# ECP-WarpX/WarpX

Measured on AMD Instinct MI355X. Metric: particle_steps_per_s, higher is better.
Workload: dtype f64; 1 GPU; 3D uniform_plasma 256x256x256, 8 ppc, Yee FDTD, order-3 shape, esirkepov, boris, filter on; cells_per_gpu=16777216, particles_per_gpu=134217728, n_ranks=1, ranks_per_gpu=1, sort_interval=2, single_precision_comms=False, preroll_steps=40, overlap_halo=False, momentum_synchronisation=outside the timed region (the K steps are consecutive steps of one longer run)

## Files before the change

### warpx_amd/csrc/common.hpp

```cpp
#ifndef WXA_COMMON_HPP_
#define WXA_COMMON_HPP_

#include <hip/hip_runtime.h>
#include <stdint.h>
#include <stdio.h>

#include "../../include/warpx_amd.h"

#ifndef WXA_OPAQUE_F64
#define WXA_OPAQUE_F64(v) asm volatile("" : "+v"(v))
#define WXA_OPAQUE_I32(v) asm volatile("" : "+v"(v))
#endif

#ifndef WXA_WAVES_PER_SIMD
#define WXA_WAVES_PER_SIMD(n) __attribute__((amdgpu_waves_per_eu(n, n)))
#endif

namespace wxa {

namespace PhysConst {
constexpr double c = 299'792'458.;
constexpr double ep0 = 8.8541878128e-12;
constexpr double mu0 = 1.25663706212e-06;
constexpr double q_e = 1.602176634e-19;
constexpr double m_e = 9.1093837015e-31;
constexpr double r_e = 2.817940326204929e-15;
}

void set_last_error(const char* fmt, ...);

#define WXA_HIP_CHECK(expr)                                                          \
    do {                                                                             \
        hipError_t _e = (expr);                                                      \
        if (_e != hipSuccess) {                                                      \
            ::wxa::set_last_error("%s failed: %s (%s:%d)", #expr, hipGetErrorString(_e), \
                                  __FILE__, __LINE__);                               \
            return WXA_ERR_HIP;                                                      \
        }                                                                            \
    } while (0)

#define WXA_LAUNCH_CHECK()                                                           \
    do {                                                                             \
        hipError_t _e = hipGetLastError();                                           \
        if (_e != hipSuccess) {                                                      \
            ::wxa::set_last_error("kernel launch failed: %s (%s:%d)", hipGetErrorString(_e), \
                                  __FILE__, __LINE__);                               \
            return WXA_ERR_HIP;                                                      \
        }                                                                            \
    } while (0)

#define WXA_REQUIRE(cond, msg)                                                       \
    do {                                                                             \
        if (!(cond)) {                                                               \
            ::wxa::set_last_error("invalid argument: %s (%s)", msg, #cond);          \
            return WXA_ERR_INVALID_ARG;                                              \
        }                                                                            \
    } while (0)

struct DevF {
    double* __restrict__ p;
    int lo0, lo1, lo2;
    int n0, n1, n2;
    long js, ks;
    __host__ __device__ inline long off(int i, int j, int k) const {
        return (long)(i - lo0) + (long)(j - lo1) * js + (long)(k - lo2) * ks;
    }
    __device__ inline double& operator()(int i, int j, int k) const { return p[off(i, j, k)]; }
};

inline DevF make_devf(const wxa_field_view& v) {
    DevF f;
    f.p = v.p;
    f.lo0 = v.lo[0]; f.lo1 = v.lo[1]; f.lo2 = v.lo[2];
    f.n0 = v.n[0]; f.n1 = v.n[1]; f.n2 = v.n[2];
    f.js = v.jstride; f.ks = v.kstride;
    return f;
}

struct Box3 {
    int lo[3];
    int hi[3];
};

inline Box3 valid_box(const wxa_field_view& v) {
    Box3 b;
    for (int d = 0; d < 3; ++d) {
        b.lo[d] = v.lo[d] + v.ng[d];
        b.hi[d] = v.lo[d] + v.n[d] - v.ng[d];
    }
    return b;
}

inline bool is_stag(const wxa_field_view& v, int a, int b, int c) {
    return v.stag[0] == a && v.stag[1] == b && v.stag[2] == c;
}
// ... 31 lines not shown
```

### warpx_amd/csrc/gather_tile.hip

```cpp
#include "dispatch.hpp"
#include "gather_body.hpp"
#include "push_sort.hpp"
#include "tile_launch.hpp"

#include <stdlib.h>

namespace wxa {

#ifdef WXA_GATHER_PROFILE
__device__ unsigned long long wxa_gather_prof[8];
#define GPROF_CLOCK(v) const long long v = clock64()
#define GPROF_ADD(n, v) do { if (threadIdx.x == 0) atomicAdd(&wxa_gather_prof[n], (unsigned long long)(v)); } while (0)
#else
#define GPROF_CLOCK(v)
#define GPROF_ADD(n, v)
#endif

constexpr int GT_TS = WXA_TILE;
constexpr int GT_THREADS = 512;

template <int G, int O = 3>
struct GatherTileDims {
    static constexpr int LO = O == 4 ? (G ? -2 : -3) : (G ? -1 : -2);
    static constexpr int N = GT_TS + (O == 4 ? (G ? 5 : 6) : (G ? 3 : 4));
    static constexpr int NPTS = N * N * N;
};

struct SplitTile {
    static constexpr int stag(int c, int d) {
        return c == 0 ? d == 0 : c == 1 ? d == 1 : c == 2 ? d == 2 : c == 3 ? d != 0 : c == 4 ? d != 1 : d != 2;
    }
    static constexpr int n(int c, int d) { return stag(c, d) ? GT_TS + 4 : GT_TS + 3; }
    static constexpr int lo(int c, int d) { return stag(c, d) ? -2 : -1; }
    static constexpr int pts(int c) { return n(c, 0) * n(c, 1) * n(c, 2); }
    static constexpr int off(int c) { return c == 0 ? 0 : off(c - 1) + pts(c - 1); }
    static constexpr int total() { return off(6); }
};

template <int N>
struct LdsField {
    const double* base;
    __device__ __forceinline__ const double* at(int i, int j, int k) const { return base + i + N * (j + N * k); }
    static constexpr long js = N, ks = N * N;
};

template <int PUSHER, bool MOVE>
__device__ __forceinline__ void push_and_store(const PV& p, int ip, double xp, double yp, double zp, double ux, double uy,
                                               double uz, double Exp, double Eyp, double Ezp, double Bxp, double Byp,
                                               double Bzp, double q, double m, double dt, const ExtEB& ext,
                                               const PushSort& hook,
                                               int* lds_hist = nullptr, const long my_tile = -1) {
    add_external_fields(ext, ip, Exp, Eyp, Ezp, Bxp, Byp, Bzp);
    push_momentum<PUSHER>(ux, uy, uz, Exp, Eyp, Ezp, Bxp, Byp, Bzp, q, m, dt);
    if constexpr (MOVE) update_position(xp, yp, zp, ux, uy, uz, dt);
    if constexpr (MOVE) {
        if (!push_sort_tail(hook, p, ip, xp, yp, zp, ux, uy, uz, lds_hist, my_tile)) return;
    }
    p.ux[ip] = ux; p.uy[ip] = uy; p.uz[ip] = uz;
    if constexpr (MOVE) { p.x[ip] = xp; p.y[ip] = yp; p.z[ip] = zp; }
}

template <int O, int G, int PUSHER, bool MOVE, int PART = 0>
__global__ void __launch_bounds__(GT_THREADS) WXA_WAVES_PER_SIMD(O <= 3 ? 4 : 2)
gather_push_tile_kernel(PV p, const int* __restrict__ offsets, DevF Ex, DevF Ey, DevF Ez, DevF Bx, DevF By,
                        DevF Bz, Geom g, TileGeom tg, double q, double m, double dt, StragglerQueue sq, ExtEB ext,
                        PushSort hook, HeavyUnits hu) {
    constexpr int N = GatherTileDims<G, O>::N;
    constexpr int NPTS = GatherTileDims<G, O>::NPTS;
    constexpr bool SPLIT = G == 0 && O <= 3;
    __shared__ double F[SPLIT ? SplitTile::total() : 6 * NPTS];
    const long ntiles = (long)tg.nt[0] * tg.nt[1] * tg.nt[2];
    if (blockIdx.x == 0 && threadIdx.x == 0 && sq.next) *sq.next = 0u;
    long tile;
    int unit_u, unit_k;
    if (!heavy_unit_of(hu, blockIdx.x, ntiles, tile, unit_u, unit_k)) return;
    constexpr int TC = GT_TS * GT_TS * GT_TS;
    int start = offsets[tile * TC];
    int end = offsets[(tile + 1) * TC];
    if (unit_k > 1) {
        const long chunks = ((long)(end - start) + 63) >> 6;
        const int s0 = start;
        start = s0 + (int)((chunks * unit_u / unit_k) << 6);
        end = min(end, s0 + (int)((chunks * (unit_u + 1) / unit_k) << 6));
    }
    if (end <= start) return;
    const int tid = threadIdx.x;
    GPROF_CLOCK(prof_t0);
    const int ti = (int)(tile % tg.nt[0]);
    const int tj = (int)((tile / tg.nt[0]) % tg.nt[1]);
    const int tk = (int)(tile / ((long)tg.nt[0] * tg.nt[1]));
    if constexpr (PART != 0) {
        const bool face = ti == 0 || ti == tg.nt[0] - 1 || tj == 0 || tj == tg.nt[1] - 1 || tk == 0 || tk == tg.nt[2] - 1;
        if (face != (PART == 2)) return;
    }
    const int o0 = tg.cell_lo[0] + ti * GT_TS + GatherTileDims<G, O>::LO;
    const int o1 = tg.cell_lo[1] + tj * GT_TS + GatherTileDims<G, O>::LO;
    const int o2 = tg.cell_lo[2] + tk * GT_TS + GatherTileDims<G, O>::LO;
    static_assert(GT_THREADS == PUSH_SORT_TILE_CELLS, "one lane per cell of the tile");
    __shared__ int lhist[MOVE ? PUSH_SORT_TILE_CELLS : 1];
    const bool count_local = MOVE && (hook.mode & PUSH_SORT_COUNT) != 0 && unit_u == 0;
    if constexpr (MOVE) {
        if (count_local) lhist[tid] = 0;
    }
    constexpr int SCAP = 512;
    __shared__ int slist[SCAP];
    __shared__ int sn, sbase;
    if (tid == 0) sn = 0;
    auto push_straggler = [&](const int i) {
        const int n = atomicAdd(&sn, 1);
        if (n < SCAP) slist[n] = i;
        else sq.push(i);
    };
    constexpr int WAVES = GT_THREADS / 64;
    __shared__ int next_chunk;
    const int lane = tid & 63;
    int cb_next = start + 64 * __builtin_amdgcn_readfirstlane(tid >> 6) + GT_THREADS;
    if (tid == 0) next_chunk = 2 * WAVES;
    int ip = start + tid;
    double nxt[3] = {0.0, 0.0, 0.0};
    auto load_particle = [&](const int i) {
        asm volatile("" ::: "memory");
        nxt[0] = p.x[i]; nxt[1] = p.y[i]; nxt[2] = p.z[i];
        asm volatile("" ::: "memory");
    };
    if (ip < end) load_particle(ip);
    constexpr int PER = (NPTS + GT_THREADS - 1) / GT_THREADS;
    auto fetch = [&](const DevF& f, double (&r)[PER]) {
#pragma unroll
        for (int n = 0; n < PER; ++n) {
            const int a = tid + n * GT_THREADS;
            const int i = o0 + a % N, j = o1 + (a / N) % N, k = o2 + a / (N * N);
            const bool in = a < NPTS && i >= f.lo0 && i < f.lo0 + f.n0 && j >= f.lo1 && j < f.lo1 + f.n1 && k >= f.lo2 &&
                            k < f.lo2 + f.n2;
            r[n] = in ? f.p[f.off(i, j, k)] : 0.0;
        }
    };
    auto put = [&](int c, const double (&r)[PER]) {
#pragma unroll
        for (int n = 0; n < PER; ++n) {
            const int a = tid + n * GT_THREADS;
            if (a < NPTS) F[c * NPTS + a] = r[n];
        }
    };
    if constexpr (SPLIT) {
        const int t0 = o0 - GatherTileDims<G, O>::LO, t1 = o1 - GatherTileDims<G, O>::LO, t2 = o2 - GatherTileDims<G, O>::LO;
        constexpr int PERS = (SplitTile::pts(3) + GT_THREADS - 1) / GT_THREADS;
        auto fetch_c = [&](auto cc, const DevF& f, double (&r)[PERS]) {
            constexpr int c = decltype(cc)::value, n0 = SplitTile::n(c, 0), n1 = SplitTile::n(c, 1);
#pragma unroll
            for (int n = 0; n < PERS; ++n) {
                const int a = tid + n * GT_THREADS;
                const int i = t0 + SplitTile::lo(c, 0) + a % n0, j = t1 + SplitTile::lo(c, 1) + (a / n0) % n1,
                          k = t2 + SplitTile::lo(c, 2) + a / (n0 * n1);
                const bool in = a < SplitTile::pts(c) && i >= f.lo0 && i < f.lo0 + f.n0 && j >= f.lo1 && j < f.lo1 + f.n1 &&
                                k >= f.lo2 && k < f.lo2 + f.n2;
                r[n] = in ? f.p[f.off(i, j, k)] : 0.0;
            }
        };
        auto put_c = [&](auto cc, const double (&r)[PERS]) {
            constexpr int c = decltype(cc)::value;
#pragma unroll
            for (int n = 0; n < PERS; ++n) {
                const int a = tid + n * GT_THREADS;
                if (a < SplitTile::pts(c)) F[SplitTile::off(c) + a] = r[n];
            }
        };
        using std::integral_constant;
        double r0[PERS], r1[PERS], r2[PERS], r3[PERS], r4[PERS], r5[PERS];
        fetch_c(integral_constant<int, 0>{}, Ex, r0); fetch_c(integral_constant<int, 1>{}, Ey, r1); fetch_c(integral_constant<int, 2>{}, Ez, r2);
        fetch_c(integral_constant<int, 3>{}, Bx, r3); fetch_c(integral_constant<int, 4>{}, By, r4); fetch_c(integral_constant<int, 5>{}, Bz, r5);
        put_c(integral_constant<int, 0>{}, r0); put_c(integral_constant<int, 1>{}, r1); put_c(integral_constant<int, 2>{}, r2);
        put_c(integral_constant<int, 3>{}, r3); put_c(integral_constant<int, 4>{}, r4); put_c(integral_constant<int, 5>{}, r5);
    } else {
        double r0[PER], r1[PER], r2[PER], r3[PER], r4[PER], r5[PER];
        fetch(Ex, r0); fetch(Ey, r1); fetch(Ez, r2); fetch(Bx, r3); fetch(By, r4); fetch(Bz, r5);
        put(0, r0); put(1, r1); put(2, r2); put(3, r3); put(4, r4); put(5, r5);
    }
    __syncthreads();
    GPROF_CLOCK(prof_t1);
    GPROF_ADD(0, prof_t1 - prof_t0);
    GPROF_ADD(2, 1);

    int claimed = 0;
    auto advance = [&]() {
        ip = cb_next + lane;
        cb_next = start + 64 * __builtin_amdgcn_readfirstlane(__shfl(claimed, 0));
    };
    for (; ip < end; advance()) {
        GPROF_CLOCK(prof_a);
        double xp = nxt[0], yp = nxt[1], zp = nxt[2], ux0, uy0, uz0;
        asm volatile("" ::: "memory");
        ux0 = p.ux[ip]; uy0 = p.uy[ip]; uz0 = p.uz[ip];
        asm volatile("" ::: "memory");
        if (lane == 0) claimed = atomicAdd(&next_chunk, 1);
        if (cb_next + lane < end) load_particle(cb_next + lane);
#ifdef WXA_GATHER_PROFILE
        asm volatile("s_waitcnt vmcnt(0)" : "+v"(xp), "+v"(yp), "+v"(zp));
#endif
        GPROF_CLOCK(prof_b);
        GatherShapes<O, G> s;
        gather_shapes<O, G>(xp, yp, zp, g, s);
        constexpr int NN = O + 1, NC = O + 1 - G;
        const int lo_i = min(s.jn, s.jc) - o0, hi_i = max(s.jn + NN, s.jc + NC) - 1 - o0;
        const int lo_j = min(s.kn, s.kc) - o1, hi_j = max(s.kn + NN, s.kc + NC) - 1 - o1;
        const int lo_k = min(s.ln, s.lc) - o2, hi_k = max(s.ln + NN, s.lc + NC) - 1 - o2;
        bool staged = lo_i >= 0 && lo_j >= 0 && lo_k >= 0 && hi_i < N && hi_j < N && hi_k < N;
        if constexpr (SPLIT) {
            staged = staged && s.jn - o0 >= 1 && s.kn - o1 >= 1 && s.ln - o2 >= 1;
        }
        if (!staged) {
            push_straggler(ip);
            continue;
        }
        const int jn = s.jn - o0, jc = s.jc - o0, kn = s.kn - o1, kc = s.kc - o1, ln = s.ln - o2, lc = s.lc - o2;
        double Exp, Eyp, Ezp, Bxp, Byp, Bzp;
        if constexpr (SPLIT) {
            auto rows = [&](auto cc, auto nx, auto ny, auto nz, const int i, const int j, const int k, const double* sx_,
                            const double* sy_, const double* sz_) {
                constexpr int c = decltype(cc)::value, n0 = SplitTile::n(c, 0), n1 = SplitTile::n(c, 1);
                const double* b_ = F + SplitTile::off(c) + (i - (SplitTile::lo(c, 0) + 2)) +
                                   n0 * ((j - (SplitTile::lo(c, 1) + 2)) + n1 * (k - (SplitTile::lo(c, 2) + 2)));
                return gather_rows_lds<decltype(nx)::value, decltype(ny)::value, decltype(nz)::value, n0, n0 * n1, 2>(b_, sx_, sy_, sz_);
            };
            using std::integral_constant;
            constexpr integral_constant<int, NN> nn{};
            constexpr integral_constant<int, NC> nc{};
            Exp = rows(integral_constant<int, 0>{}, nc, nn, nn, jc, kn, ln, s.sxc, s.syn, s.szn);
            Eyp = rows(integral_constant<int, 1>{}, nn, nc, nn, jn, kc, ln, s.sxn, s.syc, s.szn);
            Ezp = rows(integral_constant<int, 2>{}, nn, nn, nc, jn, kn, lc, s.sxn, s.syn, s.szc);
            Bzp = rows(integral_constant<int, 5>{}, nc, nc, nn, jc, kc, ln, s.sxc, s.syc, s.szn);
            Byp = rows(integral_constant<int, 4>{}, nc, nn, nc, jc, kn, lc, s.sxc, s.syn, s.szc);
            Bxp = rows(integral_constant<int, 3>{}, nn, nc, nc, jn, kc, lc, s.sxn, s.syc, s.szc);
        } else {
#define GROWS(...)                                                                                         \
    [&](const double* b_, const double* sx_, const double* sy_, const double* sz_) {                       \
         \
                                                                            \
        if constexpr (O <= 3) return gather_rows_lds<__VA_ARGS__, N, N * N, 2>(b_, sx_, sy_, sz_);        \
        else return gather_rows<__VA_ARGS__>(b_, N, N * N, sx_, sy_, sz_);                                 \
    }
            Exp = GROWS(NC, NN, NN)(F + 0 * NPTS + jc + N * (kn + N * ln), s.sxc, s.syn, s.szn);
            Eyp = GROWS(NN, NC, NN)(F + 1 * NPTS + jn + N * (kc + N * ln), s.sxn, s.syc, s.szn);
            Ezp = GROWS(NN, NN, NC)(F + 2 * NPTS + jn + N * (kn + N * lc), s.sxn, s.syn, s.szc);
            Bzp = GROWS(NC, NC, NN)(F + 5 * NPTS + jc + N * (kc + N * ln), s.sxc, s.syc, s.szn);
            Byp = GROWS(NC, NN, NC)(F + 4 * NPTS + jc + N * (kn + N * lc), s.sxc, s.syn, s.szc);
            Bxp = GROWS(NN, NC, NC)(F + 3 * NPTS + jn + N * (kc + N * lc), s.sxn, s.syc, s.szc);
#undef GROWS
        }
#ifdef WXA_GATHER_PROFILE
        double prof_e = Exp + Bxp;
        asm volatile("s_waitcnt lgkmcnt(0)" : "+v"(prof_e));
#endif
        GPROF_CLOCK(prof_c);
        push_and_store<PUSHER, MOVE>(p, ip, xp, yp, zp, ux0, uy0, uz0, Exp, Eyp, Ezp, Bxp, Byp, Bzp, q, m, dt, ext, hook,
                                     count_local ? lhist : nullptr, tile);
#ifdef WXA_GATHER_PROFILE
        asm volatile("s_waitcnt vmcnt(0)" ::: "memory");
        GPROF_CLOCK(prof_d);
        GPROF_ADD(3, prof_b - prof_a); GPROF_ADD(4, prof_c - prof_b); GPROF_ADD(5, prof_d - prof_c); GPROF_ADD(6, 1);
        if (prof_e == 1.2345e-300) p.x[ip] = prof_e;
#endif
    }
#ifdef WXA_GATHER_PROFILE
    { GPROF_CLOCK(prof_t2); GPROF_ADD(1, prof_t2 - prof_t1); }
#endif
    {
        __syncthreads();
        const int n = min(sn, SCAP);
        if (tid == 0 && n > 0) sbase = (int)atomicAdd(sq.count, (unsigned)n);
        __syncthreads();
        for (int i = tid; i < n; i += GT_THREADS) sq.idx[sbase + i] = slist[i];
    }
    if constexpr (MOVE) {
        if (count_local) {
            __syncthreads();
            push_sort_tile_finish(hook, lhist, tile, tid);
        }
    }
}

template <int O, int G, int PUSHER, bool MOVE>
__global__ void __launch_bounds__(256)
gather_push_stragglers_kernel(PV p, const int* __restrict__ idx, const unsigned* __restrict__ count, DevF Ex,
                              DevF Ey, DevF Ez, DevF Bx, DevF By, DevF Bz, Geom g, double q, double m, double dt,
                              ExtEB ext, PushSort hook) {
    const unsigned n = *count;
    for (unsigned t = blockIdx.x * blockDim.x + threadIdx.x; t < n; t += gridDim.x * blockDim.x) {
        const int ip = idx[t];
        const double xp = p.x[ip], yp = p.y[ip], zp = p.z[ip];
        GatherShapes<O, G> s;
        gather_shapes<O, G>(xp, yp, zp, g, s);
        double Exp, Eyp, Ezp, Bxp, Byp, Bzp;
        gather_global<O, G>(s, Ex, Ey, Ez, Bx, By, Bz, Exp, Eyp, Ezp, Bxp, Byp, Bzp);
        push_and_store<PUSHER, MOVE>(p, ip, xp, yp, zp, p.ux[ip], p.uy[ip], p.uz[ip], Exp, Eyp, Ezp, Bxp, Byp, Bzp, q, m, dt,
                                     ext, hook);
    }
}

wxa_status gather_push_tiled(const wxa_particle_view* p, const wxa_field_view E[3], const wxa_field_view B[3],
                             const wxa_grid_geom* geom, double q, double m, double dt, int order, int galerkin,
                             int pusher, bool move, int part, wxa_workspace* ws, hipStream_t st) {
    TileLaunch tl;
    wxa_status rc;
    if ((rc = plan_tile_launch(ws, (long)p->np, 16, ws->gather_flips, st, tl)) != WXA_OK) return rc;
    const PV pv = make_pv(*p);
    const Geom g = make_geom(*geom);
    const DevF ex = make_devf(E[0]), ey = make_devf(E[1]), ez = make_devf(E[2]);
    const DevF bx = make_devf(B[0]), by = make_devf(B[1]), bz = make_devf(B[2]);
    const ExtEB ext = ext_of(ws);
    const PushSort hook = make_push_sort(ws, 0, move);
    with_int<0, 1, 2, 3>(move ? 1 + part : 0, [&](auto what) {
    with_int<WXA_PUSHER_BORIS, WXA_PUSHER_VAY, WXA_PUSHER_HC, WXA_PUSHER_BORIS_RR>(pusher, [&](auto pu) {
    with_int<1, 2, 3, 4>(order, [&](auto o) {
    with_int<1, 0>(galerkin, [&](auto gk) {
        constexpr int O = decltype(o)::value, G = decltype(gk)::value, PUSHER = decltype(pu)::value;
        constexpr bool MOVE = decltype(what)::value != 0;
        constexpr int PART = MOVE ? decltype(what)::value - 1 : 0;
        hipLaunchKernelGGL((gather_push_tile_kernel<O, G, PUSHER, MOVE, PART>), dim3(tl.groups), dim3(GT_THREADS), 0, st, pv,
                           tl.offsets, ex, ey, ez, bx, by, bz, g, tl.tg, q, m, dt, tl.sq, ext, hook, tl.hu);
        hipLaunchKernelGGL((gather_push_stragglers_kernel<O, G, PUSHER, MOVE>), dim3(WXA_STRAGGLER_BLOCKS), dim3(256), 0, st,
                           pv, tl.sq.idx, tl.sq.count, ex, ey, ez, bx, by, bz, g, q, m, dt, ext, hook);
    }); }); }); });
    WXA_LAUNCH_CHECK();
    return WXA_OK;
}

}

#ifdef WXA_GATHER_PROFILE
extern "C" int wxa_debug_gather_profile(unsigned long long* out, int reset) {
    if (out && hipMemcpyFromSymbol(out, HIP_SYMBOL(wxa::wxa_gather_prof), sizeof(wxa::wxa_gather_prof)) != hipSuccess)
        return -1;
    if (reset) {
        unsigned long long z[8] = {};
        if (hipMemcpyToSymbol(HIP_SYMBOL(wxa::wxa_gather_prof), z, sizeof(z)) != hipSuccess) return -1;
    }
    return 0;
}
#endif
```

### warpx_amd/csrc/particles.hip

```cpp
#include "deposit_body.hpp"
#include <complex>

#include "dispatch.hpp"
#include "gather_body.hpp"
#include "push_sort.hpp"
#include "workspace.hpp"

#include <hipcub/hipcub.hpp>

namespace wxa {

template <int O, int G, int PUSHER, bool MOVE>
__global__ void __launch_bounds__(256)
gather_push_kernel(PV p, DevF Ex, DevF Ey, DevF Ez, DevF Bx, DevF By, DevF Bz, Geom g, double q,
                   double m, double dt, ExtEB ext, PushSort hook) {
    const long ip = (long)blockIdx.x * blockDim.x + threadIdx.x;
    if (ip >= p.np) return;
    double xp = p.x[ip], yp = p.y[ip], zp = p.z[ip];
    GatherShapes<O, G> s;
    gather_shapes<O, G>(xp, yp, zp, g, s);
    double Exp, Eyp, Ezp, Bxp, Byp, Bzp;
    gather_global<O, G>(s, Ex, Ey, Ez, Bx, By, Bz, Exp, Eyp, Ezp, Bxp, Byp, Bzp);

    add_external_fields(ext, ip, Exp, Eyp, Ezp, Bxp, Byp, Bzp);
    double ux = p.ux[ip], uy = p.uy[ip], uz = p.uz[ip];
    push_momentum<PUSHER>(ux, uy, uz, Exp, Eyp, Ezp, Bxp, Byp, Bzp, q, m, dt);
    if constexpr (MOVE) {
        update_position(xp, yp, zp, ux, uy, uz, dt);
        if (!push_sort_tail(hook, p, ip, xp, yp, zp, ux, uy, uz)) return;
        p.x[ip] = xp; p.y[ip] = yp; p.z[ip] = zp;
    }
    p.ux[ip] = ux; p.uy[ip] = uy; p.uz[ip] = uz;
}

__global__ void __launch_bounds__(256) lens_fields_kernel(PV p, ExtLens L, double* __restrict__ out, long stride) {
    const long ip = (long)blockIdx.x * blockDim.x + threadIdx.x;
    if (ip >= p.np) return;
    double Ex = 0., Ey = 0., Bx = 0., By = 0.;
    add_lens_fields(L, p.x[ip], p.y[ip], p.z[ip], p.ux[ip], p.uy[ip], p.uz[ip], Ex, Ey, Bx, By);
    out[ip] = Ex; out[stride + ip] = Ey; out[2 * stride + ip] = Bx; out[3 * stride + ip] = By;
}

template <int O>
__global__ void __launch_bounds__(256)
deposit_esirkepov_global_kernel(PV p, DevF Jx, DevF Jy, DevF Jz, Geom g, double q, EsirkepovStep es) {
    const long ip = (long)blockIdx.x * blockDim.x + threadIdx.x;
    if (ip >= p.np) return;
    const ParticleState ps{p.x[ip], p.y[ip], p.z[ip], p.w[ip], p.ux[ip], p.uy[ip], p.uz[ip]};
    EsirkepovShapes<O> s;
    esirkepov_shapes<O>(ps, g, q, es, s);
    GlobalSink sink = make_global_sink(Jx, Jy, Jz);
    sink.bi = s.bi; sink.bj = s.bj; sink.bk = s.bk;
    esirkepov_accumulate<O>(s, es, sink);
}

template <int O>
__global__ void __launch_bounds__(256)
deposit_direct_global_kernel(PV p, DevF Jx, DevF Jy, DevF Jz, Geom g, double q, double relative_time) {
    const long ip = (long)blockIdx.x * blockDim.x + threadIdx.x;
    if (ip >= p.np) return;
    const ParticleState ps{p.x[ip], p.y[ip], p.z[ip], p.w[ip], p.ux[ip], p.uy[ip], p.uz[ip]};
    DirectShapes<O> s;
    direct_shapes<O>(ps, g, q, relative_time, s);
    GlobalSink sink = make_global_sink(Jx, Jy, Jz);
    direct_accumulate<O>(s, sink);
}

template <int O>
__global__ void __launch_bounds__(256)
deposit_charge_kernel(PV p, DevF rho, int s0, int s1, int s2, Geom g, double q) {
    const long ip = (long)blockIdx.x * blockDim.x + threadIdx.x;
    if (ip >= p.np) return;
    const double invvol = g.dxi * g.dyi * g.dzi;
    const double wq = q * p.w[ip] * invvol;
    const double x = (p.x[ip] - g.xmin) * g.dxi;
    const double y = (p.y[ip] - g.ymin) * g.dyi;
    const double z = (p.z[ip] - g.zmin) * g.dzi;
    double sx[O + 1], sy[O + 1], sz[O + 1];
    const int i = g.lo0 + shape_factor<O>(sx, s0 ? x : x - 0.5);
    const int j = g.lo1 + shape_factor<O>(sy, s1 ? y : y - 0.5);
    const int k = g.lo2 + shape_factor<O>(sz, s2 ? z : z - 0.5);
    double* __restrict__ r = rho.p + rho.off(i, j, k);
#pragma unroll
    for (int iz = 0; iz <= O; iz++)
#pragma unroll
        for (int iy = 0; iy <= O; iy++)
#pragma unroll
            for (int ix = 0; ix <= O; ix++)
                atomic_add_f64(r + ix + iy * rho.js + iz * rho.ks, sx[ix] * sy[iy] * sz[iz] * wq);
}

__device__ __forceinline__ double wrap_periodic(double v, double plo, double phi) {
    const double L = phi - plo;
    if (v >= phi) {
        v -= L;
        if (v < plo) v = plo;
    } else if (v < plo) {
        v += L;
        if (v >= phi) v = nextafter(phi, plo);
    }
    return v;
}

struct PeriodicBox {
    double plo[3], phi[3];
    int on[3];
};

__global__ void __launch_bounds__(256)
enforce_periodic_kernel(double* __restrict__ x, double* __restrict__ y, double* __restrict__ z, long np,
                        PeriodicBox pb) {
    const long ip = (long)blockIdx.x * blockDim.x + threadIdx.x;
// ... 1023 lines not shown
```

### warpx_amd/csrc/push_sort.hpp

```cpp
#ifndef WXA_PUSH_SORT_HPP_
#define WXA_PUSH_SORT_HPP_

#include "gather_body.hpp"
#include "workspace.hpp"

namespace wxa {

struct SortGeom {
    double plo[3];
    double dinv[3];
    int nc[3];
    int retired_bin;
    int wrap[3] = {0, 0, 0};
};

__device__ __forceinline__ int cell_of(const SortGeom& s, double x, double y, double z) {
    int i = (int)floor((x - s.plo[0]) * s.dinv[0]);
    int j = (int)floor((y - s.plo[1]) * s.dinv[1]);
    int k = (int)floor((z - s.plo[2]) * s.dinv[2]);
    if (s.wrap[0]) i = i < 0 ? i + s.nc[0] : (i >= s.nc[0] ? i - s.nc[0] : i);
    if (s.wrap[1]) j = j < 0 ? j + s.nc[1] : (j >= s.nc[1] ? j - s.nc[1] : j);
    if (s.wrap[2]) k = k < 0 ? k + s.nc[2] : (k >= s.nc[2] ? k - s.nc[2] : k);
    i = min(max(i, 0), s.nc[0] - 1);
    j = min(max(j, 0), s.nc[1] - 1);
    k = min(max(k, 0), s.nc[2] - 1);
    constexpr int T = WXA_TILE;
    const int nti = (s.nc[0] + T - 1) / T, ntj = (s.nc[1] + T - 1) / T;
    const int tile = (i / T) + nti * ((j / T) + ntj * (k / T));
    const int kt = k % T;
    return tile * (T * T * T) + (i % T) + T * ((kt & 1) + 2 * ((j % T) + T * (kt >> 1)));
}

constexpr int PUSH_SORT_COUNT = WXA_PUSH_SORT_COUNT, PUSH_SORT_SCATTER = WXA_PUSH_SORT_SCATTER;
constexpr int PUSH_SORT_TILE_CELLS = WXA_TILE * WXA_TILE * WXA_TILE;
constexpr unsigned long long PUSH_SORT_FOREIGN = 0x80000000ull;

struct PushSort {
    int mode = 0;
    int check_retired = 0;
    double predict_dt = 0.0;
    long first = 0;
    SortGeom sg{};
    unsigned long long* __restrict__ kr_out = nullptr;
    int* __restrict__ hist = nullptr;
    int* __restrict__ fcnt = nullptr;
    int* __restrict__ own_out = nullptr;
    const unsigned long long* __restrict__ kr_in = nullptr;
    const int* __restrict__ offs = nullptr;
    const int* __restrict__ own_in = nullptr;
    double* __restrict__ dx = nullptr; double* __restrict__ dy = nullptr; double* __restrict__ dz = nullptr;
    double* __restrict__ dw = nullptr;
    double* __restrict__ dux = nullptr; double* __restrict__ duy = nullptr; double* __restrict__ duz = nullptr;
    unsigned long long* __restrict__ did = nullptr;
    long np_counted = 0;
    long n_appended = 0;
    int retired_bin_in = 0;
};

__device__ __forceinline__ long push_sort_dest(const PushSort& h, const long gi, bool& dropped) {
    dropped = false;
    if (gi >= h.np_counted) return (long)h.offs[h.retired_bin_in] + (gi - h.np_counted);
    const unsigned long long kr = h.kr_in[gi];
    const int key = (int)(kr >> 32);
    long d = (long)h.offs[key] + (long)(unsigned)(kr & 0x7fffffffull);
    if (kr & PUSH_SORT_FOREIGN) d += h.own_in[key];
    if (key == h.retired_bin_in) { d += h.n_appended; dropped = true; }
    return d;
}

__device__ __forceinline__ bool push_sort_tail(const PushSort& h, const PV& p, const long ip, const double xp, const double yp,
                                               const double zp, const double ux, const double uy, const double uz,
                                               int* lds_hist = nullptr, const long my_tile = -1) {
    if (h.mode == 0) return true;
    const long gi = h.first + ip;
    long at = gi;
    bool in_place = true;
    const bool scatter = (h.mode & PUSH_SORT_SCATTER) != 0;
    unsigned long long pid = 0ull;
    if (p.id && (scatter || h.check_retired)) pid = p.id[ip];
    bool dropped = false;
    if (scatter) {
        const double w = p.w[ip];
        at = push_sort_dest(h, gi, dropped);
        h.dx[at] = xp; h.dy[at] = yp; h.dz[at] = zp; h.dw[at] = w;
        h.dux[at] = ux; h.duy[at] = uy; h.duz[at] = uz;
        if (p.id && h.did) h.did[at] = pid;
        in_place = false;
    }
    if ((h.mode & PUSH_SORT_COUNT) && !dropped) {
        double kx = xp, ky = yp, kz = zp;
        if (h.predict_dt != 0.0) {
            constexpr double inv_c2 = 1.0 / (PhysConst::c * PhysConst::c);
            const double s_ = h.predict_dt / sqrt(1.0 + (ux * ux + uy * uy + uz * uz) * inv_c2);
            kx += ux * s_; ky += uy * s_; kz += uz * s_;
        }
        const int key = (h.check_retired && p.id && pid == WXA_IDCPU_RETIRED) ? h.sg.retired_bin : cell_of(h.sg, kx, ky, kz);
        unsigned long long rank;
        if (lds_hist && key / PUSH_SORT_TILE_CELLS == my_tile) {
            rank = (unsigned long long)(unsigned)atomicAdd(&lds_hist[key % PUSH_SORT_TILE_CELLS], 1);
        } else {
            rank = PUSH_SORT_FOREIGN | (unsigned long long)(unsigned)atomicAdd(&h.fcnt[key], 1);
            atomicAdd(&h.hist[key], 1);
        }
        h.kr_out[at] = ((unsigned long long)(unsigned)key << 32) | rank;
    }
    return in_place;
}

__device__ __forceinline__ void push_sort_tile_finish(const PushSort& h, const int* lds_hist, const long my_tile, const int tid) {
    const int n = lds_hist[tid];
    if (n > 0) {
        atomicAdd(&h.hist[my_tile * PUSH_SORT_TILE_CELLS + tid], n);
        h.own_out[my_tile * PUSH_SORT_TILE_CELLS + tid] = n;
    }
}

inline PushSort make_push_sort(const wxa_workspace* ws, const long first, const bool move) {
    PushSort h{};
    if (!ws || !move || ws->ps.armed == 0) return h;
    const auto& s = ws->ps;
    h.mode = s.armed;
    h.first = first;
    if (s.armed & PUSH_SORT_COUNT) {
        for (int d = 0; d < 3; ++d) { h.sg.plo[d] = s.plo[d]; h.sg.dinv[d] = s.dinv[d]; h.sg.nc[d] = s.nc[d]; h.sg.wrap[d] = s.wrap[d]; }
        h.sg.retired_bin = (int)s.bins;
        h.check_retired = s.check_retired;
        h.predict_dt = s.predict_dt;
        h.kr_out = (unsigned long long*)s.kr[s.out].p;
        h.hist = (int*)s.hist.p;
        h.fcnt = (int*)s.hist.p + (s.bins + 2);
        h.own_out = (int*)s.own[s.out].p;
    }
    if (s.armed & PUSH_SORT_SCATTER) {
        h.kr_in = (const unsigned long long*)s.kr[s.in].p;
        h.offs = (const int*)s.offs[s.in].p;
        h.own_in = (const int*)s.own[s.in].p;
        h.dx = s.dst.x; h.dy = s.dst.y; h.dz = s.dst.z; h.dw = s.dst.w;
        h.dux = s.dst.ux; h.duy = s.dst.uy; h.duz = s.dst.uz;
        h.did = (unsigned long long*)s.dst.idcpu;
        h.np_counted = s.pending_np;
        h.n_appended = s.appended;
        h.retired_bin_in = (int)s.pending_bins;
    }
    return h;
}

}
#endif
```

### warpx_amd/csrc/shapes.hpp

```cpp
#ifndef WXA_SHAPES_HPP_
#define WXA_SHAPES_HPP_

#include "common.hpp"

namespace wxa {

#define WXA_BSPLINE_BODY                                                   \
    if constexpr (ORDER == 0) {                                            \
        s[0] = 1.0;                                                        \
    } else if constexpr (ORDER == 1) {                                     \
        s[0] = 1.0 - xi;                                                   \
        s[1] = xi;                                                         \
    } else if constexpr (ORDER == 2) {                                     \
        s[0] = 0.5 * (0.5 - xi) * (0.5 - xi);                              \
        s[1] = 0.75 - xi * xi;                                             \
        s[2] = 0.5 * (0.5 + xi) * (0.5 + xi);                              \
    } else if constexpr (ORDER == 3) {                                     \
        const double om = 1.0 - xi;                                        \
        s[0] = (1.0 / 6.0) * om * om * om;                                 \
        s[1] = (2.0 / 3.0) - xi * xi * (1.0 - xi / 2.0);                   \
        s[2] = (2.0 / 3.0) - om * om * (1.0 - 0.5 * om);                   \
        s[3] = (1.0 / 6.0) * xi * xi * xi;                                 \
    } else {                     \
        static_assert(ORDER == 4, "orders 0..4");                          \
// ... 111 lines not shown
}

__device__ __forceinline__ void push_hc(double& ux, double& uy, double& uz, const double Ex, const double Ey,
                                        const double Ez, const double Bx, const double By, const double Bz,
                                        const double q, const double m, const double dt) {
    const double qmt = 0.5 * q * dt / m;
    constexpr double invclight = 1. / PhysConst::c;
    constexpr double invclightsq = 1. / (PhysConst::c * PhysConst::c);
    const double umx = ux + qmt * Ex, umy = uy + qmt * Ey, umz = uz + qmt * Ez;
    double gamma = 1. + (umx * umx + umy * umy + umz * umz) * invclightsq;
    const double betax = qmt * Bx, betay = qmt * By, betaz = qmt * Bz;
    const double betam = betax * betax + betay * betay + betaz * betaz;
    const double sigma = gamma - betam;
    const double ust = (umx * betax + umy * betay + umz * betaz) * invclight;
    gamma = 1. / sqrt(0.5 * (sigma + sqrt(sigma * sigma + 4. * (betam + ust * ust))));
    const double tx = gamma * betax, ty = gamma * betay, tz = gamma * betaz;
    const double s = 1. / (1. + (tx * tx + ty * ty + tz * tz));
    const double umt = umx * tx + umy * ty + umz * tz;
    const double upx = s * (umx + umt * tx + umy * tz - umz * ty);
    const double upy = s * (umy + umt * ty + umz * tx - umx * tz);
    const double upz = s * (umz + umt * tz + umx * ty - umy * tx);
    ux = upx + qmt * Ex + upy * tz - upz * ty;
    uy = upy + qmt * Ey + upz * tx - upx * tz;
    uz = upz + qmt * Ez + upx * ty - upy * tx;
}

__device__ __forceinline__ void push_boris_rr(double& ux, double& uy, double& uz, const double Ex, const double Ey,
                                              const double Ez, const double Bx, const double By, const double Bz,
                                              const double q, const double m, const double dt) {
    const double ux_old = ux, uy_old = uy, uz_old = uz;
    constexpr double inv_c2 = 1. / (PhysConst::c * PhysConst::c);
    push_boris(ux, uy, uz, Ex, Ey, Ez, Bx, By, Bz, q, m, dt);
    const double ux_n = (ux + ux_old) * 0.5;
    const double uy_n = (uy + uy_old) * 0.5;
    const double uz_n = (uz + uz_old) * 0.5;
    const double gamma_n = sqrt(1. + (ux_n * ux_n + uy_n * uy_n + uz_n * uz_n) * inv_c2);
    const double inv_gamma_n = 1.0 / gamma_n;
    const double vx_n = ux_n * inv_gamma_n;
    const double vy_n = uy_n * inv_gamma_n;
    const double vz_n = uz_n * inv_gamma_n;
    const double bx_n = vx_n / PhysConst::c;
    const double by_n = vy_n / PhysConst::c;
    const double bz_n = vz_n / PhysConst::c;
    const double flx_q = (Ex + vy_n * Bz - vz_n * By);
    const double fly_q = (Ey + vz_n * Bx - vx_n * Bz);
    const double flz_q = (Ez + vx_n * By - vy_n * Bx);
    const double fl_q2 = flx_q * flx_q + fly_q * fly_q + flz_q * flz_q;
    const double bdotE = (bx_n * Ex + by_n * Ey + bz_n * Ez);
    const double bdotE2 = bdotE * bdotE;
    const double coeff = gamma_n * gamma_n * (fl_q2 - bdotE2);
    const double q_over_mc = q / (m * PhysConst::c);
    const double RRcoeff = (2.0 / 3.0) * PhysConst::r_e * q_over_mc * q_over_mc;
    const double frx = RRcoeff * (PhysConst::c * (fly_q * Bz - flz_q * By) + bdotE * Ex - coeff * bx_n);
    const double fry = RRcoeff * (PhysConst::c * (flz_q * Bx - flx_q * Bz) + bdotE * Ey - coeff * by_n);
    const double frz = RRcoeff * (PhysConst::c * (flx_q * By - fly_q * Bx) + bdotE * Ez - coeff * bz_n);
    ux += frx * dt;
    uy += fry * dt;
    uz += frz * dt;
}

template <int PUSHER>
__device__ __forceinline__ void push_momentum(double& ux, double& uy, double& uz, const double Ex, const double Ey,
                                              const double Ez, const double Bx, const double By, const double Bz,
                                              const double q, const double m, const double dt) {
    if constexpr (PUSHER == WXA_PUSHER_BORIS) push_boris(ux, uy, uz, Ex, Ey, Ez, Bx, By, Bz, q, m, dt);
    else if constexpr (PUSHER == WXA_PUSHER_VAY) push_vay(ux, uy, uz, Ex, Ey, Ez, Bx, By, Bz, q, m, dt);
    else if constexpr (PUSHER == WXA_PUSHER_HC) push_hc(ux, uy, uz, Ex, Ey, Ez, Bx, By, Bz, q, m, dt);
    else push_boris_rr(ux, uy, uz, Ex, Ey, Ez, Bx, By, Bz, q, m, dt);
}

struct ExtLens {
    int n;
    double period, time, dt, gamma_boost, uz_boost;
    const double* tab;
};
struct ExtPerParticle {
    const double* fields;
    long stride;
};
struct ExtEB {
    double ex, ey, ez, bx, by, bz;
    ExtPerParticle pp;
};
__device__ __forceinline__ void add_external_fields(const ExtEB& ext, long ip, double& Ex, double& Ey, double& Ez, double& Bx,
                                                    double& By, double& Bz) {
    Ex += ext.ex; Ey += ext.ey; Ez += ext.ez; Bx += ext.bx; By += ext.by; Bz += ext.bz;
    WXA_OPAQUE_F64(Ex); WXA_OPAQUE_F64(Ey); WXA_OPAQUE_F64(Ez); WXA_OPAQUE_F64(Bx); WXA_OPAQUE_F64(By); WXA_OPAQUE_F64(Bz);
    if (ext.pp.fields) {
        Ex += ext.pp.fields[ip];
        Ey += ext.pp.fields[ext.pp.stride + ip];
        Bx += ext.pp.fields[2 * ext.pp.stride + ip];
        By += ext.pp.fields[3 * ext.pp.stride + ip];
    }
}

__device__ __forceinline__ void add_lens_fields(const ExtLens& L, const double x, const double y, const double z,
                                                const double ux, const double uy, const double uz, double& fEx,
                                                double& fEy, double& fBx, double& fBy) {
    constexpr double inv_c2 = 1. / (PhysConst::c * PhysConst::c);
    const double gamma = sqrt(1. + (ux * ux + uy * uy + uz * uz) * inv_c2);
    const double vzp = uz / gamma;
    double zl = z, zr = z + vzp * L.dt;
    if (L.gamma_boost > 1.) {
        zl = L.gamma_boost * zl + L.uz_boost * L.time;
        zr = L.gamma_boost * zr + L.uz_boost * (L.time + L.dt);
    }
    double Ex = 0., Ey = 0., Bx = 0., By = 0.;
    if (zl > 0) {
        const int i_lens = (int)floor(zl / L.period);
        if (i_lens < L.n) {
            const double lens_start = L.tab[i_lens] + i_lens * L.period;
            const double lens_end = lens_start + L.tab[L.n + i_lens];
            const double zl_bounded = fmin(fmax(zl, lens_start), lens_end);
            const double zr_bounded = fmin(fmax(zr, lens_start), lens_end);
            const double frac = (zr - zl) == 0. ? 1. : (zr_bounded - zl_bounded) / (zr - zl);
            const double sE = L.tab[2 * L.n + i_lens], sB = L.tab[3 * L.n + i_lens];
            Ex = x * frac * sE;
            Ey = y * frac * sE;
            Bx = +y * frac * sB;
            By = -x * frac * sB;
        }
    }
    if (L.gamma_boost > 1.) {
        const double Ex_boost = L.gamma_boost * Ex - L.uz_boost * By;
        const double Ey_boost = L.gamma_boost * Ey + L.uz_boost * Bx;
        const double Bx_boost = L.gamma_boost * Bx + L.uz_boost * Ey * inv_c2;
        const double By_boost = L.gamma_boost * By - L.uz_boost * Ex * inv_c2;
        Ex = Ex_boost; Ey = Ey_boost; Bx = Bx_boost; By = By_boost;
    }
    fEx += Ex; fEy += Ey; fBx += Bx; fBy += By;
}

__device__ __forceinline__ void update_position(double& x, double& y, double& z, const double ux,
                                                const double uy, const double uz, const double dt) {
    constexpr double inv_c2 = 1. / (PhysConst::c * PhysConst::c);
    const double inv_gamma = inv_sqrt(1. + (ux * ux + uy * uy + uz * uz) * inv_c2);
    x += ux * inv_gamma * dt;
    y += uy * inv_gamma * dt;
    z += uz * inv_gamma * dt;
}

struct Geom {
    double xmin, ymin, zmin;
    double dxi, dyi, dzi;
    int lo0, lo1, lo2;
};
inline Geom make_geom(const wxa_grid_geom& g) {
    return Geom{g.xyzmin[0], g.xyzmin[1], g.xyzmin[2], g.dinv[0], g.dinv[1], g.dinv[2], g.lo[0], g.lo[1], g.lo[2]};
}

}
#endif
```

Baseline: 10.51 billion particle-steps/s.

## Load rarely-used tile kernel args late from kernarg segment and specialize sort mode

Moves the external-field, straggler-queue and push-sort hook arguments of the gather/push tile kernel into a struct read through the kernarg segment pointer, loaded where used and hidden behind an opaque scalar-register barrier. The aim is to stop the compiler from hoisting these uniform values into scalar registers for the whole kernel, which reduces register pressure. It also adds a compile-time MODE parameter so the plain-push variant drops the sort tail entirely. In exchange it adds repeated scalar loads inside the particle loop, a tag check that traps on mismatch, and another template dimension that doubles the number of kernel instantiations.

```diff
diff --git a/warpx_amd/csrc/common.hpp b/warpx_amd/csrc/common.hpp
--- a/warpx_amd/csrc/common.hpp
+++ b/warpx_amd/csrc/common.hpp
@@ -11,6 +11,16 @@
 #define WXA_OPAQUE_F64(v) asm volatile("" : "+v"(v))
 #define WXA_OPAQUE_I32(v) asm volatile("" : "+v"(v))
 #endif
+
+#ifndef WXA_LATE_KERNARG
+#define WXA_LATE_KERNARG(T, first_param) ((const __attribute__((address_space(4))) T*)__builtin_amdgcn_kernarg_segment_ptr())
+#define WXA_OPAQUE_UNIFORM_PTR(p) asm volatile("" : "+s"(p))
+#else
+#define WXA_OPAQUE_UNIFORM_PTR(p) ((void)0)
+#endif
+
+constexpr unsigned long long WXA_LATE_TAG = 0x57584131004c4154ull;
+#define WXA_LATE_CHECK(p) do { if ((p)->late_tag != WXA_LATE_TAG) __builtin_trap(); } while (0)
 
 #ifndef WXA_WAVES_PER_SIMD
 #define WXA_WAVES_PER_SIMD(n) __attribute__((amdgpu_waves_per_eu(n, n)))
diff --git a/warpx_amd/csrc/gather_tile.hip b/warpx_amd/csrc/gather_tile.hip
--- a/warpx_amd/csrc/gather_tile.hip
+++ b/warpx_amd/csrc/gather_tile.hip
@@ -44,33 +44,52 @@
     static constexpr long js = N, ks = N * N;
 };
 
-template <int PUSHER, bool MOVE>
+template <int PUSHER, bool MOVE, int MODE, class E, class H>
 __device__ __forceinline__ void push_and_store(const PV& p, int ip, double xp, double yp, double zp, double ux, double uy,
                                                double uz, double Exp, double Eyp, double Ezp, double Bxp, double Byp,
-                                               double Bzp, double q, double m, double dt, const ExtEB& ext,
-                                               const PushSort& hook,
+                                               double Bzp, double q, double m, double dt, const E* ext,
+                                               const H* hook,
                                                int* lds_hist = nullptr, const long my_tile = -1) {
     add_external_fields(ext, ip, Exp, Eyp, Ezp, Bxp, Byp, Bzp);
     push_momentum<PUSHER>(ux, uy, uz, Exp, Eyp, Ezp, Bxp, Byp, Bzp, q, m, dt);
     if constexpr (MOVE) update_position(xp, yp, zp, ux, uy, uz, dt);
-    if constexpr (MOVE) {
-        if (!push_sort_tail(hook, p, ip, xp, yp, zp, ux, uy, uz, lds_hist, my_tile)) return;
+    if constexpr (MOVE && MODE != 0) {
+        if (!push_sort_tail<MODE>(hook, p, ip, xp, yp, zp, ux, uy, uz, lds_hist, my_tile)) return;
     }
     p.ux[ip] = ux; p.uy[ip] = uy; p.uz[ip] = uz;
     if constexpr (MOVE) { p.x[ip] = xp; p.y[ip] = yp; p.z[ip] = zp; }
 }
 
-template <int O, int G, int PUSHER, bool MOVE, int PART = 0>
+template <bool SORT>
+struct TileLateArgs {
+    unsigned long long late_tag = WXA_LATE_TAG;
+    ExtEB ext;
+    StragglerQueue sq;
+    PushSort hook;
+};
+template <>
+struct TileLateArgs<false> {
+    unsigned long long late_tag = WXA_LATE_TAG;
+    ExtEB ext;
+    StragglerQueue sq;
+};
+template <int O, int G, int PUSHER, bool MOVE, int PART = 0, int MODE = 0>
 __global__ void __launch_bounds__(GT_THREADS) WXA_WAVES_PER_SIMD(O <= 3 ? 4 : 2)
-gather_push_tile_kernel(PV p, const int* __restrict__ offsets, DevF Ex, DevF Ey, DevF Ez, DevF Bx, DevF By,
-                        DevF Bz, Geom g, TileGeom tg, double q, double m, double dt, StragglerQueue sq, ExtEB ext,
-                        PushSort hook, HeavyUnits hu) {
+gather_push_tile_kernel(TileLateArgs<MODE != 0> late_args, PV p, const int* __restrict__ offsets, DevF Ex, DevF Ey, DevF Ez,
+                        DevF Bx, DevF By, DevF Bz, Geom g, TileGeom tg, double q, double m, double dt, HeavyUnits hu) {
+    static_assert(MOVE || MODE == 0, "the sort is folded into pushes that move the particles");
+    static_assert(MODE == 0 || MODE == PUSH_SORT_RUNTIME, "a plain push, or the mode the hook names");
+    const auto late = WXA_LATE_KERNARG(TileLateArgs<MODE != 0>, late_args);
+    WXA_LATE_CHECK(late);
     constexpr int N = GatherTileDims<G, O>::N;
     constexpr int NPTS = GatherTileDims<G, O>::NPTS;
     constexpr bool SPLIT = G == 0 && O <= 3;
     __shared__ double F[SPLIT ? SplitTile::total() : 6 * NPTS];
     const long ntiles = (long)tg.nt[0] * tg.nt[1] * tg.nt[2];
-    if (blockIdx.x == 0 && threadIdx.x == 0 && sq.next) *sq.next = 0u;
+    if (blockIdx.x == 0 && threadIdx.x == 0) {
+        unsigned* const next = late->sq.next;
+        if (next) *next = 0u;
+    }
     long tile;
     int unit_u, unit_k;
     if (!heavy_unit_of(hu, blockIdx.x, ntiles, tile, unit_u, unit_k)) return;
@@ -98,7 +117,8 @@
     const int o2 = tg.cell_lo[2] + tk * GT_TS + GatherTileDims<G, O>::LO;
     static_assert(GT_THREADS == PUSH_SORT_TILE_CELLS, "one lane per cell of the tile");
     __shared__ int lhist[MOVE ? PUSH_SORT_TILE_CELLS : 1];
-    const bool count_local = MOVE && (hook.mode & PUSH_SORT_COUNT) != 0 && unit_u == 0;
+    bool count_local = false;
+    if constexpr (MODE != 0) count_local = (late->hook.mode & PUSH_SORT_COUNT) != 0 && unit_u == 0;
     if constexpr (MOVE) {
         if (count_local) lhist[tid] = 0;
     }
@@ -106,10 +126,10 @@
     __shared__ int slist[SCAP];
     __shared__ int sn, sbase;
     if (tid == 0) sn = 0;
-    auto push_straggler = [&](const int i) {
+    auto push_straggler = [&](const int i, const auto* la) {
         const int n = atomicAdd(&sn, 1);
         if (n < SCAP) slist[n] = i;
-        else sq.push(i);
+        else la->sq.idx[atomicAdd(la->sq.count, 1u)] = i;
     };
     constexpr int WAVES = GT_THREADS / 64;
     __shared__ int next_chunk;
@@ -187,6 +207,8 @@
         cb_next = start + 64 * __builtin_amdgcn_readfirstlane(__shfl(claimed, 0));
     };
     for (; ip < end; advance()) {
+        auto la = late;
+        WXA_OPAQUE_UNIFORM_PTR(la);
         GPROF_CLOCK(prof_a);
         double xp = nxt[0], yp = nxt[1], zp = nxt[2], ux0, uy0, uz0;
         asm volatile("" ::: "memory");
@@ -209,7 +231,7 @@
             staged = staged && s.jn - o0 >= 1 && s.kn - o1 >= 1 && s.ln - o2 >= 1;
         }
         if (!staged) {
-            push_straggler(ip);
+            push_straggler(ip, la);
             continue;
         }
         const int jn = s.jn - o0, jc = s.jc - o0, kn = s.kn - o1, kc = s.kc - o1, ln = s.ln - o2, lc = s.lc - o2;
@@ -252,8 +274,12 @@
         asm volatile("s_waitcnt lgkmcnt(0)" : "+v"(prof_e));
 #endif
         GPROF_CLOCK(prof_c);
-        push_and_store<PUSHER, MOVE>(p, ip, xp, yp, zp, ux0, uy0, uz0, Exp, Eyp, Ezp, Bxp, Byp, Bzp, q, m, dt, ext, hook,
-                                     count_local ? lhist : nullptr, tile);
+        if constexpr (MODE != 0)
+            push_and_store<PUSHER, MOVE, MODE>(p, ip, xp, yp, zp, ux0, uy0, uz0, Exp, Eyp, Ezp, Bxp, Byp, Bzp, q, m, dt, &la->ext,
+                                               &la->hook, count_local ? lhist : nullptr, tile);
+        else
+            push_and_store<PUSHER, MOVE, 0>(p, ip, xp, yp, zp, ux0, uy0, uz0, Exp, Eyp, Ezp, Bxp, Byp, Bzp, q, m, dt, &la->ext,
+                                            (const PushSort*)nullptr);
 #ifdef WXA_GATHER_PROFILE
         asm volatile("s_waitcnt vmcnt(0)" ::: "memory");
         GPROF_CLOCK(prof_d);
@@ -267,14 +293,15 @@
     {
         __syncthreads();
         const int n = min(sn, SCAP);
-        if (tid == 0 && n > 0) sbase = (int)atomicAdd(sq.count, (unsigned)n);
+        if (tid == 0 && n > 0) sbase = (int)atomicAdd(late->sq.count, (unsigned)n);
         __syncthreads();
-        for (int i = tid; i < n; i += GT_THREADS) sq.idx[sbase + i] = slist[i];
+        int* const sq_idx = late->sq.idx;
+        for (int i = tid; i < n; i += GT_THREADS) sq_idx[sbase + i] = slist[i];
     }
     if constexpr (MOVE) {
         if (count_local) {
             __syncthreads();
-            push_sort_tile_finish(hook, lhist, tile, tid);
+            if constexpr (MODE != 0) push_sort_tile_finish(&late->hook, lhist, tile, tid);
         }
     }
 }
@@ -292,8 +319,8 @@
         gather_shapes<O, G>(xp, yp, zp, g, s);
         double Exp, Eyp, Ezp, Bxp, Byp, Bzp;
         gather_global<O, G>(s, Ex, Ey, Ez, Bx, By, Bz, Exp, Eyp, Ezp, Bxp, Byp, Bzp);
-        push_and_store<PUSHER, MOVE>(p, ip, xp, yp, zp, p.ux[ip], p.uy[ip], p.uz[ip], Exp, Eyp, Ezp, Bxp, Byp, Bzp, q, m, dt,
-                                     ext, hook);
+        push_and_store<PUSHER, MOVE, PUSH_SORT_RUNTIME>(p, ip, xp, yp, zp, p.ux[ip], p.uy[ip], p.uz[ip], Exp, Eyp, Ezp, Bxp,
+                                                        Byp, Bzp, q, m, dt, &ext, &hook);
     }
 }
 
@@ -309,6 +336,7 @@
     const DevF bx = make_devf(B[0]), by = make_devf(B[1]), bz = make_devf(B[2]);
     const ExtEB ext = ext_of(ws);
     const PushSort hook = make_push_sort(ws, 0, move);
+    with_int<0, PUSH_SORT_RUNTIME>(hook.mode != 0 ? PUSH_SORT_RUNTIME : 0, [&](auto md) {
     with_int<0, 1, 2, 3>(move ? 1 + part : 0, [&](auto what) {
     with_int<WXA_PUSHER_BORIS, WXA_PUSHER_VAY, WXA_PUSHER_HC, WXA_PUSHER_BORIS_RR>(pusher, [&](auto pu) {
     with_int<1, 2, 3, 4>(order, [&](auto o) {
@@ -316,11 +344,16 @@
         constexpr int O = decltype(o)::value, G = decltype(gk)::value, PUSHER = decltype(pu)::value;
         constexpr bool MOVE = decltype(what)::value != 0;
         constexpr int PART = MOVE ? decltype(what)::value - 1 : 0;
-        hipLaunchKernelGGL((gather_push_tile_kernel<O, G, PUSHER, MOVE, PART>), dim3(tl.groups), dim3(GT_THREADS), 0, st, pv,
-                           tl.offsets, ex, ey, ez, bx, by, bz, g, tl.tg, q, m, dt, tl.sq, ext, hook, tl.hu);
+        constexpr int MODE = MOVE ? decltype(md)::value : 0;
+        TileLateArgs<MODE != 0> late;
+        late.ext = ext;
+        late.sq = tl.sq;
+        if constexpr (MODE != 0) late.hook = hook;
+        hipLaunchKernelGGL((gather_push_tile_kernel<O, G, PUSHER, MOVE, PART, MODE>), dim3(tl.groups), dim3(GT_THREADS), 0, st,
+                           late, pv, tl.offsets, ex, ey, ez, bx, by, bz, g, tl.tg, q, m, dt, tl.hu);
         hipLaunchKernelGGL((gather_push_stragglers_kernel<O, G, PUSHER, MOVE>), dim3(WXA_STRAGGLER_BLOCKS), dim3(256), 0, st,
                            pv, tl.sq.idx, tl.sq.count, ex, ey, ez, bx, by, bz, g, q, m, dt, ext, hook);
-    }); }); }); });
+    }); }); }); }); });
     WXA_LAUNCH_CHECK();
     return WXA_OK;
 }
diff --git a/warpx_amd/csrc/particles.hip b/warpx_amd/csrc/particles.hip
--- a/warpx_amd/csrc/particles.hip
+++ b/warpx_amd/csrc/particles.hip
@@ -27,7 +27,7 @@
     push_momentum<PUSHER>(ux, uy, uz, Exp, Eyp, Ezp, Bxp, Byp, Bzp, q, m, dt);
     if constexpr (MOVE) {
         update_position(xp, yp, zp, ux, uy, uz, dt);
-        if (!push_sort_tail(hook, p, ip, xp, yp, zp, ux, uy, uz)) return;
+        if (!push_sort_tail<PUSH_SORT_RUNTIME>(&hook, p, ip, xp, yp, zp, ux, uy, uz)) return;
         p.x[ip] = xp; p.y[ip] = yp; p.z[ip] = zp;
     }
     p.ux[ip] = ux; p.uy[ip] = uy; p.uz[ip] = uz;
diff --git a/warpx_amd/csrc/push_sort.hpp b/warpx_amd/csrc/push_sort.hpp
--- a/warpx_amd/csrc/push_sort.hpp
+++ b/warpx_amd/csrc/push_sort.hpp
@@ -14,22 +14,25 @@
     int wrap[3] = {0, 0, 0};
 };
 
-__device__ __forceinline__ int cell_of(const SortGeom& s, double x, double y, double z) {
-    int i = (int)floor((x - s.plo[0]) * s.dinv[0]);
-    int j = (int)floor((y - s.plo[1]) * s.dinv[1]);
-    int k = (int)floor((z - s.plo[2]) * s.dinv[2]);
-    if (s.wrap[0]) i = i < 0 ? i + s.nc[0] : (i >= s.nc[0] ? i - s.nc[0] : i);
-    if (s.wrap[1]) j = j < 0 ? j + s.nc[1] : (j >= s.nc[1] ? j - s.nc[1] : j);
-    if (s.wrap[2]) k = k < 0 ? k + s.nc[2] : (k >= s.nc[2] ? k - s.nc[2] : k);
-    i = min(max(i, 0), s.nc[0] - 1);
-    j = min(max(j, 0), s.nc[1] - 1);
-    k = min(max(k, 0), s.nc[2] - 1);
+template <class SG>
+__device__ __forceinline__ int cell_of_at(const SG* s, double x, double y, double z) {
+    const int nc0 = s->nc[0], nc1 = s->nc[1], nc2 = s->nc[2];
+    int i = (int)floor((x - s->plo[0]) * s->dinv[0]);
+    int j = (int)floor((y - s->plo[1]) * s->dinv[1]);
+    int k = (int)floor((z - s->plo[2]) * s->dinv[2]);
+    if (s->wrap[0]) i = i < 0 ? i + nc0 : (i >= nc0 ? i - nc0 : i);
+    if (s->wrap[1]) j = j < 0 ? j + nc1 : (j >= nc1 ? j - nc1 : j);
+    if (s->wrap[2]) k = k < 0 ? k + nc2 : (k >= nc2 ? k - nc2 : k);
+    i = min(max(i, 0), nc0 - 1);
+    j = min(max(j, 0), nc1 - 1);
+    k = min(max(k, 0), nc2 - 1);
     constexpr int T = WXA_TILE;
-    const int nti = (s.nc[0] + T - 1) / T, ntj = (s.nc[1] + T - 1) / T;
+    const int nti = (nc0 + T - 1) / T, ntj = (nc1 + T - 1) / T;
     const int tile = (i / T) + nti * ((j / T) + ntj * (k / T));
     const int kt = k % T;
     return tile * (T * T * T) + (i % T) + T * ((kt & 1) + 2 * ((j % T) + T * (kt >> 1)));
 }
+__device__ __forceinline__ int cell_of(const SortGeom& s, double x, double y, double z) { return cell_of_at(&s, x, y, z); }
 
 constexpr int PUSH_SORT_COUNT = WXA_PUSH_SORT_COUNT, PUSH_SORT_SCATTER = WXA_PUSH_SORT_SCATTER;
 constexpr int PUSH_SORT_TILE_CELLS = WXA_TILE * WXA_TILE * WXA_TILE;
@@ -57,61 +60,72 @@
     int retired_bin_in = 0;
 };
 
-__device__ __forceinline__ long push_sort_dest(const PushSort& h, const long gi, bool& dropped) {
+constexpr int PUSH_SORT_RUNTIME = -1;
+
+template <class H>
+__device__ __forceinline__ long push_sort_dest(const H* h, const long gi, bool& dropped) {
     dropped = false;
-    if (gi >= h.np_counted) return (long)h.offs[h.retired_bin_in] + (gi - h.np_counted);
-    const unsigned long long kr = h.kr_in[gi];
+    const long np_counted = h->np_counted;
+    const int retired_bin_in = h->retired_bin_in;
+    if (gi >= np_counted) return (long)h->offs[retired_bin_in] + (gi - np_counted);
+    const unsigned long long kr = h->kr_in[gi];
     const int key = (int)(kr >> 32);
-    long d = (long)h.offs[key] + (long)(unsigned)(kr & 0x7fffffffull);
-    if (kr & PUSH_SORT_FOREIGN) d += h.own_in[key];
-    if (key == h.retired_bin_in) { d += h.n_appended; dropped = true; }
+    long d = (long)h->offs[key] + (long)(unsigned)(kr & 0x7fffffffull);
+    if (kr & PUSH_SORT_FOREIGN) d += h->own_in[key];
+    if (key == retired_bin_in) { d += h->n_appended; dropped = true; }
     return d;
 }
 
-__device__ __forceinline__ bool push_sort_tail(const PushSort& h, const PV& p, const long ip, const double xp, const double yp,
+template <int MODE, class H>
+__device__ __forceinline__ bool push_sort_tail(const H* h, const PV& p, const long ip, const double xp, const double yp,
                                                const double zp, const double ux, const double uy, const double uz,
                                                int* lds_hist = nullptr, const long my_tile = -1) {
-    if (h.mode == 0) return true;
-    const long gi = h.first + ip;
+    const int mode = MODE == PUSH_SORT_RUNTIME ? h->mode : MODE;
+    if (mode == 0) return true;
+    const long gi = h->first + ip;
     long at = gi;
     bool in_place = true;
-    const bool scatter = (h.mode & PUSH_SORT_SCATTER) != 0;
+    const bool scatter = (mode & PUSH_SORT_SCATTER) != 0;
+    const bool check_retired = (mode & PUSH_SORT_COUNT) && h->check_retired;
     unsigned long long pid = 0ull;
-    if (p.id && (scatter || h.check_retired)) pid = p.id[ip];
+    if (p.id && (scatter || check_retired)) pid = p.id[ip];
     bool dropped = false;
     if (scatter) {
         const double w = p.w[ip];
         at = push_sort_dest(h, gi, dropped);
-        h.dx[at] = xp; h.dy[at] = yp; h.dz[at] = zp; h.dw[at] = w;
-        h.dux[at] = ux; h.duy[at] = uy; h.duz[at] = uz;
-        if (p.id && h.did) h.did[at] = pid;
+        h->dx[at] = xp; h->dy[at] = yp; h->dz[at] = zp; h->dw[at] = w;
+        h->dux[at] = ux; h->duy[at] = uy; h->duz[at] = uz;
+        unsigned long long* const did = h->did;
+        if (p.id && did) did[at] = pid;
         in_place = false;
     }
-    if ((h.mode & PUSH_SORT_COUNT) && !dropped) {
+    if ((mode & PUSH_SORT_COUNT) && !dropped) {
         double kx = xp, ky = yp, kz = zp;
-        if (h.predict_dt != 0.0) {
+        const double predict_dt = h->predict_dt;
+        if (predict_dt != 0.0) {
             constexpr double inv_c2 = 1.0 / (PhysConst::c * PhysConst::c);
-            const double s_ = h.predict_dt / sqrt(1.0 + (ux * ux + uy * uy + uz * uz) * inv_c2);
+            const double s_ = predict_dt / sqrt(1.0 + (ux * ux + uy * uy + uz * uz) * inv_c2);
             kx += ux * s_; ky += uy * s_; kz += uz * s_;
         }
-        const int key = (h.check_retired && p.id && pid == WXA_IDCPU_RETIRED) ? h.sg.retired_bin : cell_of(h.sg, kx, ky, kz);
+        const int key = (check_retired && p.id && pid == WXA_IDCPU_RETIRED) ? h->sg.retired_bin : cell_of_at(&h->sg, kx, ky, kz);
         unsigned long long rank;
         if (lds_hist && key / PUSH_SORT_TILE_CELLS == my_tile) {
             rank = (unsigned long long)(unsigned)atomicAdd(&lds_hist[key % PUSH_SORT_TILE_CELLS], 1);
         } else {
-            rank = PUSH_SORT_FOREIGN | (unsigned long long)(unsigned)atomicAdd(&h.fcnt[key], 1);
-            atomicAdd(&h.hist[key], 1);
+            rank = PUSH_SORT_FOREIGN | (unsigned long long)(unsigned)atomicAdd(&h->fcnt[key], 1);
+            atomicAdd(&h->hist[key], 1);
         }
-        h.kr_out[at] = ((unsigned long long)(unsigned)key << 32) | rank;
+        h->kr_out[at] = ((unsigned long long)(unsigned)key << 32) | rank;
     }
     return in_place;
 }
 
-__device__ __forceinline__ void push_sort_tile_finish(const PushSort& h, const int* lds_hist, const long my_tile, const int tid) {
+template <class H>
+__device__ __forceinline__ void push_sort_tile_finish(const H* h, const int* lds_hist, const long my_tile, const int tid) {
     const int n = lds_hist[tid];
     if (n > 0) {
-        atomicAdd(&h.hist[my_tile * PUSH_SORT_TILE_CELLS + tid], n);
-        h.own_out[my_tile * PUSH_SORT_TILE_CELLS + tid] = n;
+        atomicAdd(&h->hist[my_tile * PUSH_SORT_TILE_CELLS + tid], n);
+        h->own_out[my_tile * PUSH_SORT_TILE_CELLS + tid] = n;
     }
 }
 
diff --git a/warpx_amd/csrc/shapes.hpp b/warpx_amd/csrc/shapes.hpp
--- a/warpx_amd/csrc/shapes.hpp
+++ b/warpx_amd/csrc/shapes.hpp
@@ -217,16 +217,23 @@
     double ex, ey, ez, bx, by, bz;
     ExtPerParticle pp;
 };
+template <class E>
+__device__ __forceinline__ void add_external_fields(const E* ext, long ip, double& Ex, double& Ey, double& Ez, double& Bx,
+                                                    double& By, double& Bz) {
+    Ex += ext->ex; Ey += ext->ey; Ez += ext->ez; Bx += ext->bx; By += ext->by; Bz += ext->bz;
+    WXA_OPAQUE_F64(Ex); WXA_OPAQUE_F64(Ey); WXA_OPAQUE_F64(Ez); WXA_OPAQUE_F64(Bx); WXA_OPAQUE_F64(By); WXA_OPAQUE_F64(Bz);
+    const double* const fields = ext->pp.fields;
+    if (fields) {
+        const long stride = ext->pp.stride;
+        Ex += fields[ip];
+        Ey += fields[stride + ip];
+        Bx += fields[2 * stride + ip];
+        By += fields[3 * stride + ip];
+    }
+}
 __device__ __forceinline__ void add_external_fields(const ExtEB& ext, long ip, double& Ex, double& Ey, double& Ez, double& Bx,
                                                     double& By, double& Bz) {
-    Ex += ext.ex; Ey += ext.ey; Ez += ext.ez; Bx += ext.bx; By += ext.by; Bz += ext.bz;
-    WXA_OPAQUE_F64(Ex); WXA_OPAQUE_F64(Ey); WXA_OPAQUE_F64(Ez); WXA_OPAQUE_F64(Bx); WXA_OPAQUE_F64(By); WXA_OPAQUE_F64(Bz);
-    if (ext.pp.fields) {
-        Ex += ext.pp.fields[ip];
-        Ey += ext.pp.fields[ext.pp.stride + ip];
-        Bx += ext.pp.fields[2 * ext.pp.stride + ip];
-        By += ext.pp.fields[3 * ext.pp.stride + ip];
-    }
+    add_external_fields(&ext, ip, Ex, Ey, Ez, Bx, By, Bz);
 }
 
 __device__ __forceinline__ void add_lens_fields(const ExtLens& L, const double x, const double y, const double z,
```

After: 10.92 billion particle-steps/s (median of 6 runs). 3.8% higher.
